# Edward-Sun/DIFUSCO

Hardware: NVIDIA H100
Metric: TSP-500 graphs/sec, 50-step categorical denoise (higher is better)
Workload: dtype f32 (3-term bf16 split on wgmma, fp32 accumulate)

## Files before the change

difusco_b200/csrc/edge_layer_tc.cuh:

```cuda
#pragma once
#include <cuda.h>
#include <cuda_bf16.h>
#include <cuda_runtime.h>

#include <stdlib.h>

#include <string>

#include "common.cuh"
#include "edge_layer_fp32.cuh"

namespace dfb {

constexpr int WG_ROWS = 64;
constexpr int TC_KCH = 64;
constexpr int TC_B_BYTES = 256 * 128;
constexpr int TC_A_CHUNK = WG_ROWS * 128;
constexpr int TC_A_BYTES = 8 * TC_A_CHUNK;
constexpr int CONV_BATCH = 16;
constexpr int E4_BATCH = 16;

constexpr int W_LO_ROWS = H;
constexpr int W_MAT_ROWS = 2 * W_LO_ROWS;
constexpr int W_LAYER_ROWS = 6 * W_MAT_ROWS;
__host__ __device__ constexpr int w_row_C(int l) { return l * W_LAYER_ROWS; }
__host__ __device__ constexpr int w_row_O(int l) { return w_row_C(l) + W_MAT_ROWS; }
__host__ __device__ constexpr int w_row_UVAB(int l) { return w_row_C(l) + 2 * W_MAT_ROWS; }
__host__ __device__ constexpr int w_row_embed(int L, int which) { return L * W_LAYER_ROWS + which * W_MAT_ROWS; }
__host__ __device__ constexpr int w_arena_rows(int L) { return w_row_embed(L, 2); }

template <int NWG>
struct TcCfg {
  static_assert(NWG == 1 || NWG == 2, "one or two consumer warpgroups");
  static constexpr int TILE = NWG * WG_ROWS;
  static constexpr int THREADS = (NWG + 1) * 128;
  static constexpr int NSTAGE = (NWG == 1) ? 3 : 2;
  static constexpr int OFF_B = NWG * TC_A_BYTES;
  static constexpr int OFF_PRM = OFF_B + NSTAGE * TC_B_BYTES;
  static constexpr int OFF_ROW = OFF_PRM + 6 * H * 4;
  static constexpr int OFF_SRC = OFF_ROW + TILE * 4;
  static constexpr int OFF_BAR = OFF_SRC + TILE * 8;
  static constexpr int SMEM_BYTES = OFF_BAR + 2 * NSTAGE * 8;
  static constexpr int SMEM_ALLOC = SMEM_BYTES + 1024;
  static constexpr int OFF_TAU = SMEM_BYTES;
  static constexpr int SMEM_ALLOC_TROWS = SMEM_ALLOC + TILE * 8;
  static_assert(SMEM_ALLOC_TROWS <= 232448, "shared memory budget (227 KB per block)");
};

struct TcParams {
  float* e;
  const float* uvab;
  float* partials;
  GraphDev g;
  LayerParams lp;
  const float* tvec;
  const float* xt_lut;
  const float* lut;
  const float* zero_row;
  float* debug_acc;
  const float* lin_in;
  float* lin_out;
  const float* lin_bias;
  int lin_rows;
  int lin_nb;
  int lin_w_row;
  int* error_flag;
  unsigned long long* phase_cycles;
  int write_e, e_zero, agg_mode;
  int w_row_base;
  int n_tiles;
  TimeRows trows;
};

__device__ __forceinline__ uint32_t smem_u32(const void* p) { return (uint32_t)__cvta_generic_to_shared(p); }

__device__ __forceinline__ void mbar_init(uint64_t* bar, uint32_t count) {
  asm volatile("mbarrier.init.shared::cta.b64 [%0], %1;" ::"r"(smem_u32(bar)), "r"(count) : "memory");
}
__device__ __forceinline__ void mbar_arrive(uint64_t* bar) {
  asm volatile("mbarrier.arrive.shared::cta.b64 _, [%0];" ::"r"(smem_u32(bar)) : "memory");
}
__device__ __forceinline__ void mbar_arrive_expect_tx(uint64_t* bar, uint32_t bytes) {
  asm volatile("mbarrier.arrive.expect_tx.shared::cta.b64 _, [%0], %1;" ::"r"(smem_u32(bar)), "r"(bytes) : "memory");
}
__device__ __forceinline__ void mbar_wait(uint64_t* bar, uint32_t parity, int* error_flag, int code) {
  const uint32_t addr = smem_u32(bar);
  uint32_t ok = 0;
#pragma unroll 1
  for (uint32_t spin = 0;; ++spin) {
    asm volatile(
        "{\n .reg .pred p;\n mbarrier.try_wait.parity.shared::cta.b64 p, [%1], %2, %3;\n selp.u32 %0, 1, 0, p;\n}"
        : "=r"(ok)
        : "r"(addr), "r"(parity), "r"(20000u)
        : "memory");
    if (ok) return;
    if (spin > 400000u) {
      if (error_flag) {
        error_flag[1] = (int)blockIdx.x;
        error_flag[2] = (int)parity;
        error_flag[3] = (int)threadIdx.x;
        atomicExch(error_flag, code);
      }
      __threadfence_system();
      __trap();
    }
  }
}
__device__ __forceinline__ void tma_load_2d(uint32_t dst, const CUtensorMap* map, uint64_t* bar, int c0, int c1) {
  asm volatile(
      "cp.async.bulk.tensor.2d.shared::cluster.global.mbarrier::complete_tx::bytes [%0], [%1, {%3, %4}], [%2];"
      ::"r"(dst), "l"(reinterpret_cast<uint64_t>(map)), "r"(smem_u32(bar)), "r"(c0), "r"(c1)
      : "memory");
}
__device__ __forceinline__ void fence_proxy_async() { asm volatile("fence.proxy.async.shared::cta;" ::: "memory"); }

__device__ __forceinline__ uint64_t wgmma_desc_sw128(uint32_t smem_addr) {
  return (uint64_t)((smem_addr >> 4) & 0x3fffu) | (1ull << 16) | (64ull << 32) | (1ull << 62);
}
__device__ __forceinline__ void wgmma_fence() { asm volatile("wgmma.fence.sync.aligned;" ::: "memory"); }
__device__ __forceinline__ void wgmma_commit() { asm volatile("wgmma.commit_group.sync.aligned;" ::: "memory"); }
template <int N>
__device__ __forceinline__ void wgmma_wait() { asm volatile("wgmma.wait_group.sync.aligned %0;" ::"n"(N) : "memory"); }
__device__ __forceinline__ void acc_fence(float (&d)[128]) {
#pragma unroll
  for (int i = 0; i < 128; ++i) asm volatile("" : "+f"(d[i])::"memory");
}
__device__ __forceinline__ void wgmma_bf16(float (&d)[128], uint64_t da, uint64_t db, uint32_t scale_d) {
  asm volatile(
      "{\n .reg .pred p;\n setp.ne.b32 p, %130, 0;\n"
      "wgmma.mma_async.sync.aligned.m64n256k16.f32.bf16.bf16 "
      "{%0, %1, %2, %3, %4, %5, %6, %7, %8, %9, %10, %11, %12, %13, %14, %15, "
      "%16, %17, %18, %19, %20, %21, %22, %23, %24, %25, %26, %27, %28, %29, %30, %31, "
      "%32, %33, %34, %35, %36, %37, %38, %39, %40, %41, %42, %43, %44, %45, %46, %47, "
      "%48, %49, %50, %51, %52, %53, %54, %55, %56, %57, %58, %59, %60, %61, %62, %63, "
      "%64, %65, %66, %67, %68, %69, %70, %71, %72, %73, %74, %75, %76, %77, %78, %79, "
      "%80, %81, %82, %83, %84, %85, %86, %87, %88, %89, %90, %91, %92, %93, %94, %95, "
      "%96, %97, %98, %99, %100, %101, %102, %103, %104, %105, %106, %107, %108, %109, %110, %111, "
      "%112, %113, %114, %115, %116, %117, %118, %119, %120, %121, %122, %123, %124, %125, %126, %127}, "
      "%128, %129, p, 1, 1, 0, 0;\n}"
      : "+f"(d[0]), "+f"(d[1]), "+f"(d[2]), "+f"(d[3]), "+f"(d[4]), "+f"(d[5]), "+f"(d[6]), "+f"(d[7]),
        "+f"(d[8]), "+f"(d[9]), "+f"(d[10]), "+f"(d[11]), "+f"(d[12]), "+f"(d[13]), "+f"(d[14]), "+f"(d[15]),
        "+f"(d[16]), "+f"(d[17]), "+f"(d[18]), "+f"(d[19]), "+f"(d[20]), "+f"(d[21]), "+f"(d[22]), "+f"(d[23]),
        "+f"(d[24]), "+f"(d[25]), "+f"(d[26]), "+f"(d[27]), "+f"(d[28]), "+f"(d[29]), "+f"(d[30]), "+f"(d[31]),
        "+f"(d[32]), "+f"(d[33]), "+f"(d[34]), "+f"(d[35]), "+f"(d[36]), "+f"(d[37]), "+f"(d[38]), "+f"(d[39]),
        "+f"(d[40]), "+f"(d[41]), "+f"(d[42]), "+f"(d[43]), "+f"(d[44]), "+f"(d[45]), "+f"(d[46]), "+f"(d[47]),
        "+f"(d[48]), "+f"(d[49]), "+f"(d[50]), "+f"(d[51]), "+f"(d[52]), "+f"(d[53]), "+f"(d[54]), "+f"(d[55]),
        "+f"(d[56]), "+f"(d[57]), "+f"(d[58]), "+f"(d[59]), "+f"(d[60]), "+f"(d[61]), "+f"(d[62]), "+f"(d[63]),
        "+f"(d[64]), "+f"(d[65]), "+f"(d[66]), "+f"(d[67]), "+f"(d[68]), "+f"(d[69]), "+f"(d[70]), "+f"(d[71]),
        "+f"(d[72]), "+f"(d[73]), "+f"(d[74]), "+f"(d[75]), "+f"(d[76]), "+f"(d[77]), "+f"(d[78]), "+f"(d[79]),
        "+f"(d[80]), "+f"(d[81]), "+f"(d[82]), "+f"(d[83]), "+f"(d[84]), "+f"(d[85]), "+f"(d[86]), "+f"(d[87]),
        "+f"(d[88]), "+f"(d[89]), "+f"(d[90]), "+f"(d[91]), "+f"(d[92]), "+f"(d[93]), "+f"(d[94]), "+f"(d[95]),
        "+f"(d[96]), "+f"(d[97]), "+f"(d[98]), "+f"(d[99]), "+f"(d[100]), "+f"(d[101]), "+f"(d[102]), "+f"(d[103]),
        "+f"(d[104]), "+f"(d[105]), "+f"(d[106]), "+f"(d[107]), "+f"(d[108]), "+f"(d[109]), "+f"(d[110]), "+f"(d[111]),
        "+f"(d[112]), "+f"(d[113]), "+f"(d[114]), "+f"(d[115]), "+f"(d[116]), "+f"(d[117]), "+f"(d[118]), "+f"(d[119]),
        "+f"(d[120]), "+f"(d[121]), "+f"(d[122]), "+f"(d[123]), "+f"(d[124]), "+f"(d[125]), "+f"(d[126]), "+f"(d[127])
      : "l"(da), "l"(db), "r"(scale_d));
}

__device__ __forceinline__ float sigmoid_mufu(float x) {
  float t, r;
  asm("ex2.approx.ftz.f32 %0, %1;" : "=f"(t) : "f"(-1.4426950408889634f * x));
  asm("rcp.approx.ftz.f32 %0, %1;" : "=f"(r) : "f"(1.0f + t));
  return r;
}
__device__ __forceinline__ void split4(float4 x, uint2& hi, uint2& lo) {
  __nv_bfloat162 h01 = __floats2bfloat162_rn(x.x, x.y), h23 = __floats2bfloat162_rn(x.z, x.w);
  float2 f01 = __bfloat1622float2(h01), f23 = __bfloat1622float2(h23);
  __nv_bfloat162 l01 = __floats2bfloat162_rn(x.x - f01.x, x.y - f01.y);
  __nv_bfloat162 l23 = __floats2bfloat162_rn(x.z - f23.x, x.w - f23.y);
  hi.x = *reinterpret_cast<uint32_t*>(&h01);
  hi.y = *reinterpret_cast<uint32_t*>(&h23);
  lo.x = *reinterpret_cast<uint32_t*>(&l01);
  lo.y = *reinterpret_cast<uint32_t*>(&l23);
}
__device__ __forceinline__ void split2(float a, float b, uint32_t& hi, uint32_t& lo) {
  __nv_bfloat162 h = __floats2bfloat162_rn(a, b);
  const float2 f = __bfloat1622float2(h);
  __nv_bfloat162 l = __floats2bfloat162_rn(a - f.x, b - f.y);
  hi = *reinterpret_cast<uint32_t*>(&h);
  lo = *reinterpret_cast<uint32_t*>(&l);
}
__device__ __forceinline__ uint32_t sw128_off(int r, int j) {
  return (uint32_t)((r >> 3) * 1024 + (r & 7) * 128 + ((j ^ (r & 7)) << 4));
}
__device__ __forceinline__ float quad_sum(float v) {
  v += __shfl_xor_sync(0xffffffffu, v, 1);
  return v + __shfl_xor_sync(0xffffffffu, v, 2);
}
__device__ __forceinline__ void swap_row_halves(float (&d)[128]) {
#pragma unroll
  for (int j = 0; j < 32; ++j) {
    const float x0 = d[4 * j], x1 = d[4 * j + 1];
    d[4 * j] = d[4 * j + 2];
    d[4 * j + 1] = d[4 * j + 3];
    d[4 * j + 2] = x0;
    d[4 * j + 3] = x1;
  }
}

enum {
  PH_TILES = 0,
  PH_TOTAL,
  PH_CONVERT,
  PH_G1_WAIT,
  PH_G1_MMA,
  PH_E1,
  PH_REDUCE,
  PH_LN,
  PH_G2_WAIT,
  PH_G2_MMA,
  PH_E4,
  PH_COUNT
};

template <int NWG, bool LIN, bool TIMED = false, bool TROWS = false>
__device__ __forceinline__ void edge_layer_wg_body(const CUtensorMap& wmap, const TcParams& P) {
  using Cfg = TcCfg<NWG>;
  constexpr int NSTAGE = Cfg::NSTAGE;
  extern __shared__ unsigned char smem_raw[];
  unsigned char* smem = smem_raw + ((1024u - (smem_u32(smem_raw) & 1023u)) & 1023u);
  float* prm = reinterpret_cast<float*>(smem + Cfg::OFF_PRM);
  int* s_row = reinterpret_cast<int*>(smem + Cfg::OFF_ROW);
  const float** s_src = reinterpret_cast<const float**>(smem + Cfg::OFF_SRC);
  const float** s_tau = reinterpret_cast<const float**>(smem + Cfg::OFF_TAU);
  uint64_t* full = reinterpret_cast<uint64_t*>(smem + Cfg::OFF_BAR);
  uint64_t* empty = full + NSTAGE;

  const int warp = threadIdx.x >> 5, lane = threadIdx.x & 31;
  constexpr bool lin = LIN;
  const int loads_per_tile = (P.write_e ? 16 : 8) * NWG;

  if (threadIdx.x == 0) {
    for (int s = 0; s < NSTAGE; ++s) {
      mbar_init(&full[s], 1);
      mbar_init(&empty[s], 4);
    }
    asm volatile("fence.mbarrier_init.release.cluster;" ::: "memory");
    fence_proxy_async();
  }
  for (int i = threadIdx.x; i < H; i += Cfg::THREADS) {
    prm[i] = P.lp.ln_e_g[i];
    prm[H + i] = P.lp.ln_e_b[i];
    prm[2 * H + i] = P.tvec ? P.tvec[i] : 0.0f;
    prm[3 * H + i] = P.lp.ln_o_g[i];
    prm[4 * H + i] = P.lp.ln_o_b[i];
    prm[5 * H + i] = P.lp.b_O[i];
  }
  __syncthreads();
  const uint32_t smem_base = smem_u32(smem);

  if (warp >= 4 * NWG) {
    if constexpr (NWG == 2) asm volatile("setmaxnreg.dec.sync.aligned.u32 40;" ::: "memory");
    if (warp == 4 * NWG && lane == 0) {
      uint32_t u = 0;
      for (int tile = blockIdx.x; tile < P.n_tiles; tile += gridDim.x) {
        for (int i = 0; i < loads_per_tile; ++i, ++u) {
          const int s = u % NSTAGE;
          mbar_wait(&empty[s], ((u / NSTAGE) & 1) ^ 1, P.error_flag, 1);
          mbar_arrive_expect_tx(&full[s], TC_B_BYTES);
          const int row = (lin ? P.lin_w_row + (P.lin_nb == 4 ? (tile & 3) : 0) * W_MAT_ROWS
                               : P.w_row_base + (i >= 8 * NWG ? w_row_O(0) - w_row_C(0) : 0)) +
                          (i & 1) * W_LO_ROWS;
          tma_load_2d(smem_base + Cfg::OFF_B + s * TC_B_BYTES, &wmap, &full[s], ((i >> 1) & 3) * TC_KCH, row);
        }
      }
    }
    return;
  }

  if constexpr (NWG == 2) asm volatile("setmaxnreg.inc.sync.aligned.u32 232;" ::: "memory");
  const int wg = warp >> 2, wi = warp & 3, tid = threadIdx.x & 127;
  const int t4 = lane & 3;
  const int lr0 = wi * 16 + (lane >> 2);
  unsigned char* a_reg = smem + wg * TC_A_BYTES;
  const uint32_t a_base = smem_base + wg * TC_A_BYTES;
  float* msg = reinterpret_cast<float*>(a_reg);
  int* w_row = s_row + wg * WG_ROWS;
  const float** w_src = s_src + wg * WG_ROWS;
  const float** w_tau = s_tau + wg * WG_ROWS;
  auto wg_bar = [&] { asm volatile("bar.sync %0, 128;" ::"r"(1 + wg) : "memory"); };
  const int n_rows = lin ? P.lin_rows : P.g.E;
  uint32_t u = 0;
  float acc[128];

  auto turn_wait = [&] {
    if constexpr (NWG == 2) asm volatile("bar.sync %0, 256;" ::"r"(3 + wg) : "memory");
  };
  auto turn_pass = [&] {
    if constexpr (NWG == 2) asm volatile("bar.arrive %0, 256;" ::"r"(4 - wg) : "memory");
  };
  if (wg == 1) turn_pass();

  uint32_t t_mark = 0, t_start = 0;
  if constexpr (TIMED) t_start = t_mark = (uint32_t)clock();
  auto record = [&](int slot, uint32_t v) {
    if constexpr (TIMED) {
      if (tid == 0) atomicAdd(P.phase_cycles + slot, (unsigned long long)v);
    }
  };
  auto mark = [&](int slot) {
    if constexpr (TIMED) {
      const uint32_t now = (uint32_t)clock();
      record(slot, now - t_mark);
      t_mark = now;
    }
  };

  auto gemm = [&](int wait_slot, int mma_slot) {
    uint32_t waited = 0;
    turn_wait();
    if constexpr (TIMED) t_mark = (uint32_t)clock();
    acc_fence(acc);
    wgmma_fence();
    int s_prev = 0;
#pragma unroll
    for (int i = 0; i < 8; ++i, ++u) {
      const int s = u % NSTAGE;
      uint32_t w0 = 0;
      if constexpr (TIMED) w0 = (uint32_t)clock();
      mbar_wait(&full[s], (u / NSTAGE) & 1, P.error_flag, 2);
      if constexpr (TIMED) waited += (uint32_t)clock() - w0;
      const uint32_t b = smem_base + Cfg::OFF_B + s * TC_B_BYTES;
      const uint32_t ahi = a_base + (i >> 1) * 2 * TC_A_CHUNK, alo = ahi + TC_A_CHUNK;
#pragma unroll
      for (int ks = 0; ks < 4; ++ks) {
        const uint64_t db = wgmma_desc_sw128(b + ks * 32);
        wgmma_bf16(acc, wgmma_desc_sw128(ahi + ks * 32), db, (i | ks) ? 1u : 0u);
        if ((i & 1) == 0) wgmma_bf16(acc, wgmma_desc_sw128(alo + ks * 32), db, 1u);
      }
      wgmma_commit();
      if (i > 0) {
        wgmma_wait<1>();
        __syncwarp();
        if (lane == 0) mbar_arrive(&empty[s_prev]);
      }
      s_prev = s;
    }
    wgmma_wait<0>();
    acc_fence(acc);
    __syncwarp();
    if (lane == 0) mbar_arrive(&empty[s_prev]);
    turn_pass();
    if constexpr (TIMED) {
      const uint32_t now = (uint32_t)clock();
      record(wait_slot, waited);
      record(mma_slot, now - t_mark - waited);
      t_mark = now;
    }
  };

  for (int tile = blockIdx.x; tile < P.n_tiles; tile += gridDim.x) {
    record(PH_TILES, 1);
    const int row_tile = (lin && P.lin_nb == 4) ? (tile >> 2) : tile;
    const int s_base = row_tile * Cfg::TILE + wg * WG_ROWS;
    if (tid < WG_ROWS) {
      const int s = s_base + tid;
      const float* src = P.zero_row;
      int rw = -1;
      if (s < n_rows && lin) {
        src = P.lin_in + (size_t)s * H;
      } else if (s < n_rows) {
        rw = P.g.row[s];
        if (P.e_zero) src = P.zero_row;
        else if (P.xt_lut) src = P.lut + ((P.xt_lut[P.g.perm ? P.g.perm[s] : s] != 0.0f) ? H : 0);
        else src = P.e + (size_t)s * H;
      }
      w_row[tid] = rw;
      w_src[tid] = src;
      if constexpr (TROWS) w_tau[tid] = s < n_rows ? time_row(P.tvec, P.trows, P.g.perm ? P.g.perm[s] : s) : P.zero_row;
    }
    wg_bar();

#pragma unroll 1
    for (int it0 = 0; it0 < 32; it0 += CONV_BATCH) {
      float4 x[CONV_BATCH];
#pragma unroll
      for (int q = 0; q < CONV_BATCH; ++q) {
        const int item = (it0 + q) * 128 + tid;
        x[q] = __ldcg(reinterpret_cast<const float4*>(w_src[item >> 6]) + (item & 63));
      }
#pragma unroll
      for (int q = 0; q < CONV_BATCH; ++q) {
        const int item = (it0 + q) * 128 + tid;
        const int rr = item >> 6, k4 = item & 63;
        uint2 hi, lo;
        split4(x[q], hi, lo);
        const uint32_t off = (k4 >> 4) * 2 * TC_A_CHUNK + sw128_off(rr, (k4 & 15) >> 1) + (k4 & 1) * 8;
        *reinterpret_cast<uint2*>(a_reg + off) = hi;
        *reinterpret_cast<uint2*>(a_reg + off + TC_A_CHUNK) = lo;
      }
    }
    fence_proxy_async();
    wg_bar();
    mark(PH_CONVERT);
    gemm(PH_G1_WAIT, PH_G1_MMA);

    const int sa = s_base + lr0, sb = sa + 8;
    const bool va = sa < n_rows, vb = sb < n_rows;
    if (lin || P.debug_acc) {
      const int nb = (lin && P.lin_nb == 4) ? (tile & 3) : 0;
      const int ostride = lin ? P.lin_nb * H : H;
      float* out = lin ? P.lin_out + nb * H : P.debug_acc;
#pragma unroll
      for (int h = 0; h < 2; ++h) {
        const int s = h ? sb : sa;
        if (!(h ? vb : va)) continue;
#pragma unroll
        for (int j = 0; j < 32; ++j) {
          const int c = 8 * j + 2 * t4;
          float2 o = make_float2(acc[4 * j + 2 * h], acc[4 * j + 2 * h + 1]);
          if (lin) {
            const float2 bb = __ldg(reinterpret_cast<const float2*>(P.lin_bias + nb * H + c));
            o.x += bb.x;
            o.y += bb.y;
          }
          __stcg(reinterpret_cast<float2*>(out + (size_t)s * ostride + c), o);
        }
      }
      continue;
    }

    const float* src_a = w_src[lr0];
    const float* src_b = w_src[lr0 + 8];
#pragma unroll 1
    for (int h = 0; h < 2; ++h) {
      const int s = h ? sb : sa;
      const bool v = h ? vb : va;
      const float* cp = P.uvab + (size_t)(v ? P.g.col[s] : 0) * 4 * H;
      const float* rp = P.uvab + (size_t)(v ? P.g.row[s] : 0) * 4 * H + 3 * H;
      const int r = lr0 + 8 * h;
#pragma unroll
      for (int j = 0; j < 32; ++j) {
        const int c = 8 * j + 2 * t4;
        const float2 ah = __ldg(reinterpret_cast<const float2*>(cp + 2 * H + c));
        const float2 vh = __ldg(reinterpret_cast<const float2*>(cp + H + c));
        const float2 bh = __ldg(reinterpret_cast<const float2*>(rp + c));
        const float x0 = (acc[4 * j] + ah.x) + bh.x;
        const float x1 = (acc[4 * j + 1] + ah.y) + bh.y;
        acc[4 * j] = x0;
        acc[4 * j + 1] = x1;
        *reinterpret_cast<float2*>(msg + r * H + (c ^ (8 * (r & 7)))) =
            make_float2(sigmoid_mufu(x0) * vh.x, sigmoid_mufu(x1) * vh.y);
      }
      swap_row_halves(acc);
    }
    wg_bar();
    mark(PH_E1);
    const bool amax = P.agg_mode == AGG_MAX;
    const float run0 = amax ? -INFINITY : 0.0f;
#pragma unroll 1
    for (int g2 = 0; g2 < WG_ROWS / GROUP; ++g2) {
      const int grp = (s_base >> 5) + g2;
      if (grp >= P.g.n_groups) break;
      const int first_node = P.g.grp_first[grp];
      const size_t pair_base = (size_t)P.g.grp_pair[grp];
      const int node = w_row[g2 * GROUP + lane];
      const int nxt = __shfl_down_sync(0xffffffffu, node, 1);
      const uint32_t ends = __ballot_sync(0xffffffffu, node >= 0 && (lane == GROUP - 1 || nxt != node));
#pragma unroll 1
      for (int cc = 0; cc < 2; ++cc) {
        const int c = tid + 128 * cc;
        float run = run0;
#pragma unroll 8
        for (int r = 0; r < GROUP; ++r) {
          const int lr = g2 * GROUP + r;
          const float m = msg[lr * H + (c ^ (8 * (lr & 7)))];
          run = amax ? fmaxf(run, m) : run + m;
          if ((ends >> r) & 1u) {
            P.partials[(pair_base + (size_t)(w_row[lr] - first_node)) * H + c] = run;
            run = run0;
          }
        }
      }
    }
    wg_bar();
    mark(PH_REDUCE);
    if (!P.write_e) continue;

#pragma unroll 1
    for (int h = 0; h < 2; ++h) {
      float sum = 0.f;
#pragma unroll
      for (int j = 0; j < 32; ++j) sum += acc[4 * j] + acc[4 * j + 1];
      float mean = quad_sum(sum) * (1.0f / H);
      float q = 0.f;
#pragma unroll
      for (int j = 0; j < 32; ++j) {
        const float d0 = acc[4 * j] - mean, d1 = acc[4 * j + 1] - mean;
        q = fmaf(d0, d0, fmaf(d1, d1, q));
      }
      float rstd = rsqrtf(quad_sum(q) * (1.0f / H) + LN_EPS);
      sum = 0.f;
      const float* tau = nullptr;
      if constexpr (TROWS) tau = w_tau[lr0 + 8 * h];
#pragma unroll
      for (int j = 0; j < 32; ++j) {
        const int c = 8 * j + 2 * t4;
        const float2 g = *reinterpret_cast<const float2*>(prm + c);
        const float2 b = *reinterpret_cast<const float2*>(prm + H + c);
        float2 t;
        if constexpr (TROWS) t = __ldg(reinterpret_cast<const float2*>(tau + c));
        else t = *reinterpret_cast<const float2*>(prm + 2 * H + c);
        const float y0 = fmaxf(fmaf((acc[4 * j] - mean) * rstd, g.x, b.x), 0.0f) + t.x;
        const float y1 = fmaxf(fmaf((acc[4 * j + 1] - mean) * rstd, g.y, b.y), 0.0f) + t.y;
        acc[4 * j] = y0;
        acc[4 * j + 1] = y1;
        sum += y0 + y1;
      }
      mean = quad_sum(sum) * (1.0f / H);
      q = 0.f;
#pragma unroll
      for (int j = 0; j < 32; ++j) {
        const float d0 = acc[4 * j] - mean, d1 = acc[4 * j + 1] - mean;
        q = fmaf(d0, d0, fmaf(d1, d1, q));
      }
      rstd = rsqrtf(quad_sum(q) * (1.0f / H) + LN_EPS);
      const int r = lr0 + 8 * h;
#pragma unroll
      for (int j = 0; j < 32; ++j) {
        const int c = 8 * j + 2 * t4;
        const float2 g = *reinterpret_cast<const float2*>(prm + 3 * H + c);
        const float2 b = *reinterpret_cast<const float2*>(prm + 4 * H + c);
        const float z0 = fmaf((acc[4 * j] - mean) * rstd, g.x, b.x);
        const float z1 = fmaf((acc[4 * j + 1] - mean) * rstd, g.y, b.y);
        uint32_t hi, lo;
        split2(z0 * sigmoid_mufu(z0), z1 * sigmoid_mufu(z1), hi, lo);
        const uint32_t off = (j >> 3) * 2 * TC_A_CHUNK + sw128_off(r, j & 7) + 4 * t4;
        *reinterpret_cast<uint32_t*>(a_reg + off) = hi;
        *reinterpret_cast<uint32_t*>(a_reg + off + TC_A_CHUNK) = lo;
      }
      swap_row_halves(acc);
    }
    fence_proxy_async();
    wg_bar();
    mark(PH_LN);
    gemm(PH_G2_WAIT, PH_G2_MMA);

#pragma unroll
    for (int h = 0; h < 2; ++h) {
      if (!(h ? vb : va)) continue;
      const float* src = h ? src_b : src_a;
      float* dst = P.e + (size_t)(h ? sb : sa) * H;
#pragma unroll
      for (int j0 = 0; j0 < 32; j0 += E4_BATCH) {
        float2 ein[E4_BATCH];
#pragma unroll
        for (int q = 0; q < E4_BATCH; ++q) ein[q] = __ldcg(reinterpret_cast<const float2*>(src + 8 * (j0 + q) + 2 * t4));
#pragma unroll
        for (int q = 0; q < E4_BATCH; ++q) {
          const int j = j0 + q, c = 8 * j + 2 * t4;
          const float2 bo = *reinterpret_cast<const float2*>(prm + 5 * H + c);
          __stcg(reinterpret_cast<float2*>(dst + c),
                 make_float2((ein[q].x + acc[4 * j + 2 * h]) + bo.x, (ein[q].y + acc[4 * j + 2 * h + 1]) + bo.y));
        }
      }
    }
    mark(PH_E4);
  }
  if constexpr (TIMED) record(PH_TOTAL, (uint32_t)clock() - t_start);
}

__global__ void __launch_bounds__(TcCfg<2>::THREADS, 1)
k_edge_layer_wg2(const __grid_constant__ CUtensorMap wmap, const TcParams P) {
  edge_layer_wg_body<2, false>(wmap, P);
}
__global__ void __launch_bounds__(TcCfg<2>::THREADS, 1)
k_edge_layer_wg2_timed(const __grid_constant__ CUtensorMap wmap, const TcParams P) {
  edge_layer_wg_body<2, false, true>(wmap, P);
}
__global__ void __launch_bounds__(TcCfg<1>::THREADS, 1)
k_edge_layer_wg1(const __grid_constant__ CUtensorMap wmap, const TcParams P) {
  edge_layer_wg_body<1, false>(wmap, P);
}
__global__ void __launch_bounds__(TcCfg<2>::THREADS, 1)
k_edge_layer_wg2_trows(const __grid_constant__ CUtensorMap wmap, const TcParams P) {
  edge_layer_wg_body<2, false, false, true>(wmap, P);
}
__global__ void __launch_bounds__(TcCfg<1>::THREADS, 1)
k_edge_layer_wg1_trows(const __grid_constant__ CUtensorMap wmap, const TcParams P) {
  edge_layer_wg_body<1, false, false, true>(wmap, P);
}
__global__ void __launch_bounds__(TcCfg<2>::THREADS, 1)
k_linear_wg2(const __grid_constant__ CUtensorMap wmap, const TcParams P) {
  edge_layer_wg_body<2, true>(wmap, P);
}

struct TcState {
  std::string err;
  int num_sms = 0;
  CUtensorMap wmap;
  bool bound = false;
  float* zero_row = nullptr;
  int* error_flag = nullptr;
  int* error_host = nullptr;
  unsigned long long* phase_cycles = nullptr;

  TcState() = default;
  TcState(const TcState&) = delete;
  TcState& operator=(const TcState&) = delete;
  ~TcState() {
    if (zero_row) cudaFree(zero_row);
    if (error_host) cudaFreeHost(error_host);
    if (phase_cycles) cudaFree(phase_cycles);
  }
};

typedef CUresult (*PFN_encodeTiled)(CUtensorMap*, CUtensorMapDataType, cuuint32_t, void*, const cuuint64_t*,
                                    const cuuint64_t*, const cuuint32_t*, const cuuint32_t*, CUtensorMapInterleave,
                                    CUtensorMapSwizzle, CUtensorMapL2promotion, CUtensorMapFloatOOBfill);

inline int tc_init(TcState* st, int num_sms) {
  st->num_sms = num_sms;
  cudaError_t e = cudaFuncSetAttribute(k_edge_layer_wg2, cudaFuncAttributeMaxDynamicSharedMemorySize, TcCfg<2>::SMEM_ALLOC);
  if (e == cudaSuccess)
    e = cudaFuncSetAttribute(k_edge_layer_wg2_timed, cudaFuncAttributeMaxDynamicSharedMemorySize, TcCfg<2>::SMEM_ALLOC);
  if (e == cudaSuccess)
    e = cudaFuncSetAttribute(k_edge_layer_wg1, cudaFuncAttributeMaxDynamicSharedMemorySize, TcCfg<1>::SMEM_ALLOC);
  if (e == cudaSuccess)
    e = cudaFuncSetAttribute(k_edge_layer_wg2_trows, cudaFuncAttributeMaxDynamicSharedMemorySize, TcCfg<2>::SMEM_ALLOC_TROWS);
  if (e == cudaSuccess)
    e = cudaFuncSetAttribute(k_edge_layer_wg1_trows, cudaFuncAttributeMaxDynamicSharedMemorySize, TcCfg<1>::SMEM_ALLOC_TROWS);
  if (e == cudaSuccess)
    e = cudaFuncSetAttribute(k_linear_wg2, cudaFuncAttributeMaxDynamicSharedMemorySize, TcCfg<2>::SMEM_ALLOC);
  if (e != cudaSuccess) {
    st->err = std::string("cudaFuncSetAttribute: ") + cudaGetErrorString(e);
    return -2;
  }
  if ((e = cudaMalloc(&st->zero_row, H * sizeof(float))) != cudaSuccess ||
      (e = cudaMemset(st->zero_row, 0, H * sizeof(float))) != cudaSuccess ||
      (e = cudaMalloc(&st->phase_cycles, 32 * sizeof(unsigned long long))) != cudaSuccess ||
      (e = cudaMemset(st->phase_cycles, 0, 32 * sizeof(unsigned long long))) != cudaSuccess ||
      (e = cudaHostAlloc(&st->error_host, 4 * sizeof(int), cudaHostAllocMapped)) != cudaSuccess ||
      (e = cudaHostGetDevicePointer((void**)&st->error_flag, st->error_host, 0)) != cudaSuccess) {
    st->err = std::string("tc_init alloc: ") + cudaGetErrorString(e);
    return -2;
  }
  return 0;
}

inline int tc_bind_weights(TcState* st, const uint16_t* arena, int L) {
  void* fn = nullptr;
  cudaDriverEntryPointQueryResult qres;
  cudaError_t e = cudaGetDriverEntryPoint("cuTensorMapEncodeTiled", &fn, cudaEnableDefault, &qres);
  if (e != cudaSuccess || !fn || qres != cudaDriverEntryPointSuccess) {
    st->err = "cuTensorMapEncodeTiled entry point not available";
    cudaGetLastError();
    return -2;
  }
  cuuint64_t gdim[2] = {(cuuint64_t)H, (cuuint64_t)w_arena_rows(L)};
  cuuint64_t gstride[1] = {(cuuint64_t)H * sizeof(uint16_t)};
  cuuint32_t box[2] = {(cuuint32_t)TC_KCH, 256u};
  cuuint32_t estr[2] = {1u, 1u};
  CUresult r = ((PFN_encodeTiled)fn)(&st->wmap, CU_TENSOR_MAP_DATA_TYPE_BFLOAT16, 2, (void*)arena, gdim,
                                     gstride, box, estr, CU_TENSOR_MAP_INTERLEAVE_NONE, CU_TENSOR_MAP_SWIZZLE_128B,
                                     CU_TENSOR_MAP_L2_PROMOTION_L2_256B, CU_TENSOR_MAP_FLOAT_OOB_FILL_NONE);
  if (r != CUDA_SUCCESS) {
    st->err = "cuTensorMapEncodeTiled failed with CUresult " + std::to_string((int)r);
    return -2;
  }
  st->bound = true;
  return 0;
}

template <int NWG>
inline int tc_launch(TcState* st, void (*kernel)(CUtensorMap, TcParams), TcParams& P, int rows, int nb,
                     cudaStream_t stream, int smem = TcCfg<NWG>::SMEM_ALLOC) {
  if (!st->bound) {
    st->err = "weights not bound";
    return -1;
  }
  P.zero_row = st->zero_row; P.error_flag = st->error_flag; P.phase_cycles = st->phase_cycles;
  P.n_tiles = nb * ((rows + TcCfg<NWG>::TILE - 1) / TcCfg<NWG>::TILE);
  const int grid = P.n_tiles < st->num_sms ? P.n_tiles : st->num_sms;
  kernel<<<grid, TcCfg<NWG>::THREADS, smem, stream>>>(st->wmap, P);
  const cudaError_t err = cudaGetLastError();
  if (err == cudaSuccess) return 0;
  st->err = std::string("launch: ") + cudaGetErrorString(err);
  return -2;
}

inline int tc_launch_edge_layer(TcState* st, int l, float* e, const float* uvab, float* partials, const GraphDev& g,
                                const LayerParams& lp, const float* tvec, const TimeRows& trows, int write_e,
                                int e_zero, const float* xt_lut, const float* lut, int agg_mode, int nwg, bool timed,
                                float* debug_acc, cudaStream_t stream) {
  TcParams P{};
  P.e = e; P.uvab = uvab; P.partials = partials; P.g = g; P.lp = lp; P.tvec = tvec;
  P.xt_lut = xt_lut; P.lut = lut; P.debug_acc = debug_acc;
  P.write_e = debug_acc ? 0 : write_e;
  P.e_zero = e_zero; P.agg_mode = agg_mode;
  P.w_row_base = w_row_C(l);
  if (trows.index && tvec && !debug_acc) {
    P.trows = trows;
    if (nwg == 1) return tc_launch<1>(st, k_edge_layer_wg1_trows, P, g.E, 1, stream, TcCfg<1>::SMEM_ALLOC_TROWS);
    return tc_launch<2>(st, k_edge_layer_wg2_trows, P, g.E, 1, stream, TcCfg<2>::SMEM_ALLOC_TROWS);
  }
  if (nwg == 1) return tc_launch<1>(st, k_edge_layer_wg1, P, g.E, 1, stream);
  return tc_launch<2>(st, timed && !debug_acc ? k_edge_layer_wg2_timed : k_edge_layer_wg2, P, g.E, 1, stream);
}

inline int tc_launch_linear(TcState* st, const float* in, float* out, const float* bias, int rows, int nb, int w_row,
                            cudaStream_t stream) {
  TcParams P{};
  P.lin_in = in; P.lin_out = out; P.lin_bias = bias; P.lin_rows = rows; P.lin_nb = nb; P.lin_w_row = w_row;
  P.lp.ln_e_g = P.lp.ln_e_b = P.lp.ln_o_g = P.lp.ln_o_b = P.lp.b_O = st->zero_row;
  return tc_launch<2>(st, k_linear_wg2, P, rows, nb, stream);
}

}
```

Before: 20.43.

## Stage gathered V rows and residual edge rows into shared memory via cp.async

Replaces the per-thread scattered float2 __ldg gathers of the V vectors (epilogue 1) and the __ldcg residual edge-row loads (epilogue 4) with warp-cooperative 16-byte cp.async copies into the swizzled msg shared buffer. For V, the copies are issued before the A/B bias adds so they overlap that work, and the sigmoid gate is then applied in place in shared memory. The aim is fully coalesced row loads and fewer outstanding global requests per thread. In exchange it adds cp.async waits and warp syncs, reuses the msg buffer for the residual after GEMM2, and depends on the swizzle in the new msg_col helper matching the layout the stage_rows copies write.

```diff
diff --git a/difusco_b200/csrc/edge_layer_tc.cuh b/difusco_b200/csrc/edge_layer_tc.cuh
--- a/difusco_b200/csrc/edge_layer_tc.cuh
+++ b/difusco_b200/csrc/edge_layer_tc.cuh
@@ -18,7 +18,6 @@
 constexpr int TC_A_CHUNK = WG_ROWS * 128;
 constexpr int TC_A_BYTES = 8 * TC_A_CHUNK;
 constexpr int CONV_BATCH = 16;
-constexpr int E4_BATCH = 16;
 
 constexpr int W_LO_ROWS = H;
 constexpr int W_MAT_ROWS = 2 * W_LO_ROWS;
@@ -113,6 +112,11 @@
       : "memory");
 }
 __device__ __forceinline__ void fence_proxy_async() { asm volatile("fence.proxy.async.shared::cta;" ::: "memory"); }
+__device__ __forceinline__ void cp_async16(void* dst, const void* src) {
+  asm volatile("cp.async.cg.shared.global [%0], [%1], 16;" ::"r"(smem_u32(dst)), "l"(src) : "memory");
+}
+__device__ __forceinline__ void cp_async_commit() { asm volatile("cp.async.commit_group;" ::: "memory"); }
+__device__ __forceinline__ void cp_async_wait_all() { asm volatile("cp.async.wait_group 0;" ::: "memory"); }
 
 __device__ __forceinline__ uint64_t wgmma_desc_sw128(uint32_t smem_addr) {
   return (uint64_t)((smem_addr >> 4) & 0x3fffu) | (1ull << 16) | (64ull << 32) | (1ull << 62);
@@ -183,6 +187,7 @@
 __device__ __forceinline__ uint32_t sw128_off(int r, int j) {
   return (uint32_t)((r >> 3) * 1024 + (r & 7) * 128 + ((j ^ (r & 7)) << 4));
 }
+__device__ __forceinline__ int msg_col(int j, int r) { return 64 * (j >> 3) + ((8 * (j & 7)) ^ (8 * (r & 7))); }
 __device__ __forceinline__ float quad_sum(float v) {
   v += __shfl_xor_sync(0xffffffffu, v, 1);
   return v + __shfl_xor_sync(0xffffffffu, v, 2);
@@ -347,6 +352,18 @@
       record(mma_slot, now - t_mark - waited);
       t_mark = now;
     }
+  };
+
+  auto stage_rows = [&](auto row_src) {
+#pragma unroll 1
+    for (int i = 0; i < 16; ++i) {
+      const int r = wi * 16 + i;
+      const float* src = row_src(i) + 4 * lane;
+      float* dst = msg + r * H + ((4 * lane) ^ (8 * (r & 7)));
+      cp_async16(dst, src);
+      cp_async16(dst + 128, src + 128);
+    }
+    cp_async_commit();
   };
 
   for (int tile = blockIdx.x; tile < P.n_tiles; tile += gridDim.x) {
@@ -420,27 +437,32 @@
       continue;
     }
 
-    const float* src_a = w_src[lr0];
-    const float* src_b = w_src[lr0 + 8];
+    const int s_lane = s_base + wi * 16 + (lane & 15);
+    const int col_lane = s_lane < n_rows ? P.g.col[s_lane] : 0;
+    stage_rows([&](int i) { return P.uvab + (size_t)__shfl_sync(0xffffffffu, col_lane, i) * 4 * H + H; });
 #pragma unroll 1
     for (int h = 0; h < 2; ++h) {
-      const int s = h ? sb : sa;
       const bool v = h ? vb : va;
-      const float* cp = P.uvab + (size_t)(v ? P.g.col[s] : 0) * 4 * H;
-      const float* rp = P.uvab + (size_t)(v ? P.g.row[s] : 0) * 4 * H + 3 * H;
-      const int r = lr0 + 8 * h;
+      const float* ap = P.uvab + (size_t)__shfl_sync(0xffffffffu, col_lane, (lane >> 2) + 8 * h) * 4 * H + 2 * H;
+      const float* bp = P.uvab + (size_t)(v ? P.g.row[h ? sb : sa] : 0) * 4 * H + 3 * H;
 #pragma unroll
       for (int j = 0; j < 32; ++j) {
         const int c = 8 * j + 2 * t4;
-        const float2 ah = __ldg(reinterpret_cast<const float2*>(cp + 2 * H + c));
-        const float2 vh = __ldg(reinterpret_cast<const float2*>(cp + H + c));
-        const float2 bh = __ldg(reinterpret_cast<const float2*>(rp + c));
-        const float x0 = (acc[4 * j] + ah.x) + bh.x;
-        const float x1 = (acc[4 * j + 1] + ah.y) + bh.y;
-        acc[4 * j] = x0;
-        acc[4 * j + 1] = x1;
-        *reinterpret_cast<float2*>(msg + r * H + (c ^ (8 * (r & 7)))) =
-            make_float2(sigmoid_mufu(x0) * vh.x, sigmoid_mufu(x1) * vh.y);
+        const float2 ah = __ldg(reinterpret_cast<const float2*>(ap + c));
+        const float2 bh = __ldg(reinterpret_cast<const float2*>(bp + c));
+        acc[4 * j] = (acc[4 * j] + ah.x) + bh.x;
+        acc[4 * j + 1] = (acc[4 * j + 1] + ah.y) + bh.y;
+      }
+      if (h == 0) {
+        cp_async_wait_all();
+        __syncwarp();
+      }
+      float* m = msg + (lr0 + 8 * h) * H + 2 * t4;
+#pragma unroll
+      for (int j = 0; j < 32; ++j) {
+        float2* mp = reinterpret_cast<float2*>(m + msg_col(j, lr0));
+        const float2 vh = *mp;
+        *mp = make_float2(sigmoid_mufu(acc[4 * j]) * vh.x, sigmoid_mufu(acc[4 * j + 1]) * vh.y);
       }
       swap_row_halves(acc);
     }
@@ -531,28 +553,30 @@
       }
       swap_row_halves(acc);
     }
+    const float* e_src = w_src[wi * 16 + (lane & 15)];
     fence_proxy_async();
     wg_bar();
     mark(PH_LN);
     gemm(PH_G2_WAIT, PH_G2_MMA);
 
+    stage_rows([&](int i) {
+      return reinterpret_cast<const float*>(__shfl_sync(0xffffffffu, reinterpret_cast<unsigned long long>(e_src), i));
+    });
+    cp_async_wait_all();
+    __syncwarp();
 #pragma unroll
     for (int h = 0; h < 2; ++h) {
       if (!(h ? vb : va)) continue;
-      const float* src = h ? src_b : src_a;
+      const int r = lr0 + 8 * h;
+      const float* er = msg + r * H + 2 * t4;
       float* dst = P.e + (size_t)(h ? sb : sa) * H;
 #pragma unroll
-      for (int j0 = 0; j0 < 32; j0 += E4_BATCH) {
-        float2 ein[E4_BATCH];
-#pragma unroll
-        for (int q = 0; q < E4_BATCH; ++q) ein[q] = __ldcg(reinterpret_cast<const float2*>(src + 8 * (j0 + q) + 2 * t4));
-#pragma unroll
-        for (int q = 0; q < E4_BATCH; ++q) {
-          const int j = j0 + q, c = 8 * j + 2 * t4;
-          const float2 bo = *reinterpret_cast<const float2*>(prm + 5 * H + c);
-          __stcg(reinterpret_cast<float2*>(dst + c),
-                 make_float2((ein[q].x + acc[4 * j + 2 * h]) + bo.x, (ein[q].y + acc[4 * j + 2 * h + 1]) + bo.y));
-        }
+      for (int j = 0; j < 32; ++j) {
+        const int c = 8 * j + 2 * t4;
+        const float2 ein = *reinterpret_cast<const float2*>(er + msg_col(j, r));
+        const float2 bo = *reinterpret_cast<const float2*>(prm + 5 * H + c);
+        __stcg(reinterpret_cast<float2*>(dst + c),
+               make_float2((ein.x + acc[4 * j + 2 * h]) + bo.x, (ein.y + acc[4 * j + 2 * h + 1]) + bo.y));
       }
     }
     mark(PH_E4);
```

Result: faster. 22.35 (median of 6 runs) (+9.4%).
